# quartiq/stabilizer-stream

Measured on AMD Instinct MI355X. Metric: MS/s ingested (PsdCascade N=1024, raw f32), higher is better.
Workload: dtype f32

## Files before the change

stabilizer-stream_amd/csrc/fused.hip:

```cpp
#include <algorithm>
#include <cmath>
#include <cstdlib>
#include <type_traits>
#include <vector>

#include <hip/hip_ext.h>

#include "fft_block.h"
#include "fft_team.h"
#include "frames.h"
#include "fused_common.h"

#ifndef PSDK_HOIST_LOOKAHEAD
#define PSDK_HOIST_LOOKAHEAD 1
#endif
#ifndef PSDK_UADDR
#define PSDK_UADDR 1
#endif
#ifndef PSDK_ULOOP
#define PSDK_ULOOP 1
#endif

namespace psdk {

#ifdef PSDK_STAMPS
__device__ unsigned long long g_stamps[16];
#define PSDK_STAMP(k)                                                \
    do {                                                             \
        if (stamp_on) {                                              \
            const unsigned long long t_ = __builtin_amdgcn_s_memtime(); \
            st[k] += t_ - tprev;                                     \
            tprev = t_;                                              \
        }                                                            \
    } while (0)
#else
#define PSDK_STAMP(k) \
    do {              \
    } while (0)
#endif

#ifndef PSDK_ABL
#define PSDK_ABL 0
#endif

template <int N>
struct FusedGeo : FusedDec<N> {
    using T = TeamFft<N>;
    static constexpr int TEAM = T::TEAM, TPW = T::TPW;
    static constexpr int TEAMS = FUSED_WAVES * TPW;
    static constexpr int SCR = 2 * T::FRAME;
    static_assert(FusedDec<N>::END <= SCR && FusedDec<N>::WEND <= SCR, "decimator arrays exceed the frame");
    static constexpr size_t LDS_BYTES = sizeof(cf) * (TEAMS * T::FRAME + T::TW0_SIZE + T::TW1_SIZE) +
                                        sizeof(float) * (N + TEAMS * FusedDec<N>::HIST);
};

template <int TEAM>
__device__ __forceinline__ float team_bcast(float v, int team_lane0, int tl)
{
    if constexpr (TEAM == 64)
        return __builtin_bit_cast(float, __builtin_amdgcn_readlane(__builtin_bit_cast(int, v), tl));
    else
        return __shfl(v, team_lane0 + tl, 64);
}

template <class P>
__device__ __forceinline__ P *wave_uniform(P *p)
{
    const uintptr_t a = reinterpret_cast<uintptr_t>(p);
    const unsigned lo = __builtin_amdgcn_readfirstlane((unsigned)a);
    const unsigned hi = __builtin_amdgcn_readfirstlane((unsigned)(a >> 32));
    return reinterpret_cast<P *>((uintptr_t)hi << 32 | lo);
}

__device__ __forceinline__ void addtid_st2(unsigned m0, int dwa, float xa, int dwb, float xb)
{
    unsigned keep;
    asm volatile("s_mov_b32 %0, m0\n\t"
                 "s_mov_b32 m0, %1\n\t"
                 "s_nop 0\n\t"
                 "ds_write_addtid_b32 %2 offset:%4\n\t"
                 "ds_write_addtid_b32 %3 offset:%5\n\t"
                 "s_mov_b32 m0, %0"
                 : "=&s"(keep)
                 : "s"(m0), "v"(xa), "v"(xb), "i"(4 * dwa), "i"(4 * dwb)
                 : "memory");
}

template <int TEAM>
__device__ __forceinline__ float team_sum(float v)
{
    if constexpr (TEAM == 64)
        return wave_sum64(v);
    v = row_sum16(v);
    if constexpr (TEAM == 32)
        v += __shfl_xor(v, 16, 64);
    return v;
}

#ifndef PSDK_EWMA_WPS
#define PSDK_EWMA_WPS FUSED_WAVES_PER_SIMD
#endif
#ifndef PSDK_FOLD
#define PSDK_FOLD 1
#endif
#if PSDK_FOLD
template <int THREADS>
__device__ __forceinline__ void fused_aux_role(const FusedAux &aux, int b, double *scratch)
{
    constexpr int SLICES = 32, BINS = THREADS / SLICES;
    static_assert(BINS == AUX_RED_BINS, "the host sizes the aux grid by AUX_RED_BINS");
    const int n = aux.n, lane = threadIdx.x % BINS, slice = threadIdx.x / BINS;
    const int tall_blocks = aux.nred_tall * aux.red_xb, mid_blocks = aux.nred_mid * aux.red_mb;
    if (b < tall_blocks) {
        const RedJob &job = aux.red[b / aux.red_xb];
        const int k = (b % aux.red_xb) * BINS + lane;
        const bool live = k <= n / 2;
        double acc = 0.0;
        if (live) {
            const int km = k ? n - k : 0;
            int t = slice;
            for (; t + 3 * SLICES < job.nparts; t += 4 * SLICES) {
                float v[4][2];
#pragma unroll
                for (int u = 0; u < 4; ++u) {
                    const float *p = job.partial + (size_t)(t + u * SLICES) * n;
                    v[u][0] = p[k];
                    v[u][1] = p[km];
                }
#pragma unroll
                for (int u = 0; u < 4; ++u)
                    acc += (double)v[u][0] + (double)v[u][1];
            }
            for (; t < job.nparts; t += SLICES) {
                const float *p = job.partial + (size_t)t * n;
                acc += (double)p[k] + (double)p[km];
            }
        }
        scratch[slice * (BINS + 1) + lane] = acc;
        __syncthreads();
        if (slice == 0 && live) {
            acc = 0.0;
#pragma unroll
            for (int i = 0; i < SLICES; ++i)
                acc += scratch[i * (BINS + 1) + lane];
            job.spectrum[k] = job.g_total * job.spectrum[k] + (float)(0.5 * acc);
        }
        return;
    }
    b -= tall_blocks;
    if (b < mid_blocks) {
        const RedJob &job = aux.red[aux.nred_tall + b / aux.red_mb];
        const int g0 = (b % aux.red_mb) * AUX_MID_GROUPS;
        float v[AUX_MID_GROUPS][2][2];
        const bool r0 = slice < job.nparts, r1 = slice + SLICES < job.nparts;
#pragma unroll
        for (int g = 0; g < AUX_MID_GROUPS; ++g) {
            const int k = (g0 + g) * BINS + lane;
            if (k <= n / 2) {
                const int km = k ? n - k : 0;
                if (r0) {
                    v[g][0][0] = job.partial[(size_t)slice * n + k];
                    v[g][0][1] = job.partial[(size_t)slice * n + km];
                }
                if (r1) {
                    v[g][1][0] = job.partial[(size_t)(slice + SLICES) * n + k];
                    v[g][1][1] = job.partial[(size_t)(slice + SLICES) * n + km];
                }
            }
        }
#pragma unroll
        for (int g = 0; g < AUX_MID_GROUPS; ++g) {
            double acc = 0.0;
            if ((g0 + g) * BINS + lane <= n / 2) {
                if (r0)
                    acc += (double)v[g][0][0] + (double)v[g][0][1];
                if (r1)
                    acc += (double)v[g][1][0] + (double)v[g][1][1];
            }
            scratch[(g * SLICES + slice) * (BINS + 1) + lane] = acc;
        }
        __syncthreads();
        const int k = (g0 + slice) * BINS + lane;
        if (slice < AUX_MID_GROUPS && k <= n / 2) {
            double acc = 0.0;
#pragma unroll
            for (int i = 0; i < SLICES; ++i)
                acc += scratch[(slice * SLICES + i) * (BINS + 1) + lane];
            job.spectrum[k] = job.g_total * job.spectrum[k] + (float)(0.5 * acc);
        }
        return;
    }
    b -= mid_blocks;
    if (b < aux.nred - aux.nred_tall - aux.nred_mid) {
        const RedJob &job = aux.red[aux.nred_tall + aux.nred_mid + b];
        for (int k = threadIdx.x; k <= n / 2; k += THREADS) {
            const int km = k ? n - k : 0;
            float v[AUX_SHORT_ROWS][2];
#pragma unroll
            for (int t = 0; t < AUX_SHORT_ROWS; ++t)
                if (t < job.nparts) {
                    v[t][0] = job.partial[(size_t)t * n + k];
                    v[t][1] = job.partial[(size_t)t * n + km];
                }
            double acc = 0.0;
#pragma unroll
            for (int t = 0; t < AUX_SHORT_ROWS; ++t)
                if (t < job.nparts)
                    acc += (double)v[t][0] + (double)v[t][1];
            job.spectrum[k] = job.g_total * job.spectrum[k] + (float)(0.5 * acc);
        }
        return;
    }
    const TailJob &job = aux.tail[b - (aux.nred - aux.nred_tall - aux.nred_mid)];
    for (int i = threadIdx.x; i < job.count; i += THREADS)
        job.dst[i] = job.src[i];
}
#define PSDK_FOLD_PARAM , const FusedAux aux
#ifndef PSDK_AUX_BACK
#define PSDK_AUX_BACK 0
#endif
#ifndef PSDK_PRE_SCOPE
#define PSDK_PRE_SCOPE "workgroup"
#endif
#else
#define PSDK_FOLD_PARAM
#endif

template <int N, int DETREND, bool EWMA, bool FRAMES = false, int SINGLE = 0>
__global__ __launch_bounds__(FUSED_WAVES * 64, EWMA ? PSDK_EWMA_WPS : FUSED_WAVES_PER_SIMD) void fused_kernel(
    const FusedBatch batch, const float *__restrict__ win PSDK_FOLD_PARAM)
{
    using G = FusedGeo<N>;
    using T = TeamFft<N>;
    constexpr int TEAM = G::TEAM, TPW = G::TPW, TEAMS = G::TEAMS;
    __shared__ __attribute__((aligned(16))) cf s_frames[TEAMS * T::FRAME];
    __shared__ cf s_tw0[T::TW0_SIZE];
    __shared__ cf s_tw1[T::TW1_SIZE > 0 ? T::TW1_SIZE : 1];
    __shared__ float4 s_win[N / 4];
    __shared__ float s_hist[TEAMS * G::HIST];

#if PSDK_FOLD
#if PSDK_AUX_BACK
    if ((int)blockIdx.x >= batch.nblocks) {
        fused_aux_role<FUSED_WAVES * 64>(aux, (int)blockIdx.x - batch.nblocks, reinterpret_cast<double *>(s_frames));
        return;
    }
#else
    if ((int)blockIdx.x < aux.nblocks) {
        fused_aux_role<FUSED_WAVES * 64>(aux, (int)blockIdx.x, reinterpret_cast<double *>(s_frames));
        return;
    }
#endif
#endif
#ifdef PSDK_STAMPS
    const unsigned long long t_entry = __builtin_amdgcn_s_memtime();
#endif
    const int tid = threadIdx.x;
    const int lane = tid & 63, wv = tid >> 6;
    const int tm = lane / TEAM, tl = lane % TEAM;
    const int team = wv * TPW + tm;

    for (int i = tid; i < T::TW0_SIZE; i += FUSED_WAVES * 64) {
        const int c = i / TEAM, l = i % TEAM;
        float sn, cs;
        sincospif(-2.0f * (float)(4 * l + c) / (float)N, &sn, &cs);
        s_tw0[i] = {cs, sn};
    }
    for (int i = tid; i < T::TW1_SIZE; i += FUSED_WAVES * 64) {
        const int q = i / 16 + 1, s = i % 16;
        float sn, cs;
        sincospif(-2.0f * (float)(s * q) / (float)T::L1, &sn, &cs);
        s_tw1[i] = {cs, sn};
    }
    for (int i = tid; i < N / 4; i += FUSED_WAVES * 64)
        s_win[i] = *reinterpret_cast<const float4 *>(win + 4 * i);

#if PSDK_FOLD && !PSDK_AUX_BACK
    int bid = (int)blockIdx.x - aux.nblocks;
#else
    int bid = blockIdx.x;
#endif
    if constexpr (FRAMES) {
        for (int g = 0; g < batch.n_fgroups; ++g) {
            const int b0 = batch.fg_begin[g], nb = batch.fg_nb[g];
            if (bid >= b0 && bid < b0 + 4 * nb) {
                const int p = bid - b0, full = (nb >> 3) * 32;
                int c, w;
                if (p < full) {
                    c = (p >> 3) & 3;
                    w = (p >> 5) * 8 + (p & 7);
                } else {
                    const int rem = nb & 7, q_ = p - full;
                    c = q_ / rem;
                    w = (nb & ~7) + q_ % rem;
                }
                bid = b0 + c * nb + w;
                break;
            }
        }
    }
    const int ji = job_of_unit(batch, bid, [](const FusedJob &j) { return j.block_begin; });
    const FusedJob &job = batch.jobs[ji];
    const int wb = bid - job.block_begin;
    const int npairs = job.npairs, run = job.run;
#if PSDK_FOLD
    const bool has_pre = job.pre_count != 0;
    if (has_pre) {
        for (int q = 0; q < job.pre_count; ++q) {
            const TailJob &t = aux.tail[job.pre_first + q];
            for (int i = tid; i < t.count; i += FUSED_WAVES * 64)
                t.dst[i] = t.src[i];
        }
        __builtin_amdgcn_fence(__ATOMIC_RELEASE, PSDK_PRE_SCOPE);
    }
#endif

    cf *frame = s_frames + team * T::FRAME;
    float *sf = reinterpret_cast<float *>(frame);
    float *hs = s_hist + team * G::HIST;
    const unsigned m0f = T::PLANES ? T::lds_base(frame) : 0u;
    if constexpr (T::PLANES) {
        if (T::lds_base(s_frames + (TEAMS - 1) * T::FRAME) >= T::M0_LIMIT)
            __builtin_trap();
    }

    const float ta[HBF_MA] = {PSDK_HBF_TAPS_A};
    const float tb[HBF_MB] = {PSDK_HBF_TAPS_B};
    const float tc[HBF_MC] = {PSDK_HBF_TAPS_C};

    constexpr int HR = (G::HIST + TEAM - 1) / TEAM;
    unsigned h_pack[HR];
#pragma unroll
    for (int r = 0; r < HR; ++r)
        h_pack[r] = G::hist_slot(tl + TEAM * r);

    float q[16];
#pragma unroll
    for (int s = 0; s < 16; ++s)
        q[s] = 0.0f;

    __syncthreads();
#if PSDK_FOLD
    if (has_pre)
        __builtin_amdgcn_fence(__ATOMIC_ACQUIRE, PSDK_PRE_SCOPE);
#endif
#ifdef PSDK_STAMPS
    const bool stamp_on = wb == 0 && run >= 8 && tid < 64;
    unsigned long long st[12] = {0, 0, 0, 0, 0, 0, 0, 0, 0, 0, 0, 0};
    unsigned long long tprev = __builtin_amdgcn_s_memtime();
    st[9] = tprev - t_entry;
#endif

    constexpr bool UNI = TEAM == 64 && !FRAMES;
    constexpr bool UADDR = UNI && PSDK_UADDR != 0, ULOOP = UNI && PSDK_ULOOP != 0;
    const int p0 = ULOOP ? __builtin_amdgcn_readfirstlane((wb * TEAMS + team) * run) : (wb * TEAMS + team) * run;
    const int nrun = min(run, npairs - p0);
    const bool act0 = nrun > 0;
    unsigned voff = UADDR ? 16u * (unsigned)tl : 0u, voff_o = UADDR ? 8u * (unsigned)tl : 0u;
    const float4 *cp = UADDR ? wave_uniform(reinterpret_cast<const float4 *>(job.src) + (size_t)p0 * (N / 4) + N / 4)
                             : reinterpret_cast<const float4 *>(job.src) + (size_t)p0 * (N / 4) + tl;
    auto lane_off = [](unsigned &v) {
        asm volatile("" : "+v"(v));
        return v;
    };
    auto ld4 = [](const float4 *c, int k, unsigned vo) -> float4 {
        typedef float f4v __attribute__((ext_vector_type(4)));
        const f4v r = *(const __attribute__((address_space(1))) f4v *)(reinterpret_cast<const char *>(c + (k - N / 4)) + vo);
        return make_float4(r.x, r.y, r.z, r.w);
    };
    const bool fr = FRAMES && job.fspan >= 0;
    const FrameSpan &fsp = batch.fspans[fr ? job.fspan : 0];
    const unsigned ch_off = fr ? (unsigned)job.fch * 16u : 0u;
    const unsigned dac_flip = (fr && job.fch >= 2) ? 0x80008000u : 0u;
    const __amdgpu_buffer_rsrc_t rsrc = __builtin_amdgcn_make_buffer_rsrc(
        const_cast<uint8_t *>(fsp.frames), 0, fr ? (int)min(fsp.bytes, 0x7FFFFFFFull) : 0, 0x00020000);
    unsigned sp = job.s_off + (unsigned)p0 * N + 4u * tl;
    using G4 = Grp4<FRAMES>;
    auto piece = [&](const float4 *c, unsigned s_, int k) -> G4 {
        G4 g;
        if constexpr (FRAMES) {
            if (fr) {
                const unsigned si = s_ + 4u * (unsigned)k;
                const unsigned off = frame_cell_offset(fsp, si >> 3) + ch_off + (si & 4u) * 2u;
                const auto r = __builtin_amdgcn_raw_buffer_load_b64(rsrc, off, 0, 0);
                g.set_raw((unsigned)r[0], (unsigned)r[1]);
                return g;
            }
        }
        if constexpr (UADDR)
            g.set(ld4(c, k, voff));
        else
            g.set(c[k]);
        return g;
    };
    auto volts = [&](G4 &g) {
        if constexpr (FRAMES) {
            if (fr)
                grp_volts(g, dac_flip, adcdac_lsb());
        }
    };
    const float4 *safe = act0 ? cp : reinterpret_cast<const float4 *>(job.src) + (UADDR ? N / 4 : tl);
    if constexpr (UADDR && !ULOOP)
        safe = wave_uniform(safe);
    unsigned safe_s = act0 ? sp : job.s_off + 4u * tl;
    G4 ga[2], gb[2], gc[2];
    {
        const float4 z4 = make_float4(0.f, 0.f, 0.f, 0.f);
        ga[0].set(z4), ga[1].set(z4), gb[0].set(z4), gb[1].set(z4), gc[0].set(z4), gc[1].set(z4);
    }
    if (act0) {
        ga[0] = piece(cp, sp, 0);
        ga[1] = piece(cp, sp, TEAM);
        gb[0] = piece(cp, sp, 2 * TEAM);
        gb[1] = piece(cp, sp, 3 * TEAM);
        gc[0] = piece(cp, sp, N / 4);
        gc[1] = piece(cp, sp, N / 4 + TEAM);
        volts(ga[0]);
        volts(ga[1]);
        volts(gb[0]);
        volts(gb[1]);
        volts(gc[0]);
        volts(gc[1]);
    }

    {
        const float *xn = job.src + (size_t)p0 * N + N / 2;
        const long long lim = -(long long)job.pre - ((long long)p0 * N + N / 2);
        for (int r = tl; r < G::WX / 2; r += TEAM) {
            const int i0 = 2 * r - G::WX;
            float e = 0.0f, o = 0.0f;
            if (act0 && i0 >= lim) {
                if (fr) {
                    const unsigned long long si = (unsigned long long)((long long)job.s_off + (long long)p0 * N + N / 2 + i0);
                    e = frame_sample(fsp, job.fch, si);
                    o = frame_sample(fsp, job.fch, si + 1);
                } else {
                    e = xn[i0];
                    o = xn[i0 + 1];
                }
            }
            sf[G::WXE + r] = e;
            sf[G::WXO + r] = o;
        }
        wave_sync();
        for (int u = tl; u < G::WA / 2; u += TEAM) {
            float y0, y1;
            hbf_two<HBF_MA, G::A_CE, G::A_CO>(sf + G::WXE, sf + G::WXO, 2 * u, ta, y0, y1);
            sf[G::WAE + u] = y0;
            sf[G::WAO + u] = y1;
            if (u >= G::WA / 2 - 11) {
                hs[u - (G::WA / 2 - 11)] = y0;
                hs[11 + u - (G::WA / 2 - 11)] = y1;
            }
        }
        wave_sync();
        for (int u = tl; u < G::WB / 2; u += TEAM) {
            float y0, y1;
            hbf_two<HBF_MB, G::B_CE, G::B_CO>(sf + G::WAE, sf + G::WAO, 2 * u, tb, y0, y1);
            hs[22 + u] = y0;
            hs[51 + u] = y1;
        }
        wave_sync();
    }

    constexpr bool HREG = HR <= 3;
    float hreg[HR];
#pragma unroll
    for (int r = 0; r < HR; ++r)
        hreg[r] = (HREG && tl + TEAM * r < G::HIST) ? hs[tl + TEAM * r] : 0.0f;
    float piv = 0.0f, s0c = 0.0f;
    if constexpr (DETREND == 3) {
        auto r4 = [](const float4 &x) { return (x.x + x.y) + (x.z + x.w); };
        piv = team_sum<TEAM>((r4(ga[0].f()) + r4(ga[1].f())) + (r4(gb[0].f()) + r4(gb[1].f()))) * (1.0f / (float)N);
        auto s4 = [](const float4 &x, float pv) { return ((x.x - pv) + (x.y - pv)) + ((x.z - pv) + (x.w - pv)); };
        s0c = team_sum<TEAM>(s4(ga[0].f(), piv) + s4(ga[1].f(), piv));
    }
    EwmaAmp eamp;
    if constexpr (EWMA) {
        if (job.ewma)
            eamp.init(job, job.step0 + (SINGLE != 0 ? 1 : 2) * p0);
    }
    PSDK_STAMP(10);
    float keep[16];
#pragma unroll
    for (int s = 0; s < 16; ++s)
        keep[s] = 0.0f;
    auto pair_step = [&](G4(&glo)[2], G4(&gup)[2], G4(&gnl)[2], const float4 *cnext, unsigned snext, bool more,
                         float *o, int p, auto odd_step) {
        constexpr bool DOUBLE = SINGLE == 2, ODD = decltype(odd_step)::value;
        float4 lo[2] = {glo[0].f(), glo[1].f()}, up[2] = {gup[0].f(), gup[1].f()};
        const float4 nl[2] = {gnl[0].f(), gnl[1].f()};
        PSDK_STAMP(0);
#ifdef PSDK_STAMPS
        if constexpr (TEAM == 64) {
            asm volatile("s_waitcnt vmcnt(0)" ::: "memory");
            PSDK_STAMP(1);
        }
#endif
        __builtin_amdgcn_s_setprio(PSDK_DEC_PRIO);
        if constexpr (!(PSDK_ABL & 4)) {
        if constexpr (!(PSDK_ABL & 2)) {
#pragma unroll
        for (int r = 0; r < HR; ++r)
            if ((h_pack[r] & 0xFFFFu) != 0xFFFFu)
                sf[h_pack[r] & 0xFFFFu] = HREG ? hreg[r] : hs[tl + TEAM * r];
        }
        if constexpr (PSDK_ABL & 16) {
        } else if constexpr (TEAM == 64) {
            const float4 *pc[5] = {&lo[1], &up[0], &up[1], &nl[0], &nl[1]};
            float p1y = dpp_shr1(0.0f, pc[0]->y), p1w = dpp_shr1(0.0f, pc[0]->w);
            float p2w = dpp_shr1(0.0f, p1w);
#pragma unroll
            for (int r = 0; r < 4; ++r) {
                const float4 &pv = *pc[r], &cu = *pc[r + 1];
                const float s1x = dpp_shr1(dpp_ror1(pv.x), cu.x), s1y = dpp_shr1(dpp_ror1(pv.y), cu.y);
                const float s1z = dpp_shr1(dpp_ror1(pv.z), cu.z), s1w = dpp_shr1(dpp_ror1(pv.w), cu.w);
                const float s2y = dpp_shr1(dpp_ror1(p1y), s1y), s2w = dpp_shr1(dpp_ror1(p1w), s1w);
                const float s3w = dpp_shr1(dpp_ror1(p2w), s2w);
                float a0 = 0.0f, a1 = 0.0f;
                a0 += (s3w + cu.y) * ta[0];
                a1 += (s2y + cu.w) * ta[0];
                a0 += (s2y + s1w) * ta[1];
                a1 += (s2w + cu.y) * ta[1];
                a0 += (s2w + s1y) * ta[2];
                a1 += (s1y + s1w) * ta[2];
                if constexpr (T::PLANES) {
                    addtid_st2(m0f, G::AE + 11 + TEAM * r, s1x + a0, G::AO + 11 + TEAM * r, s1z + a1);
                } else {
                    const int u = tl + TEAM * r;
                    sf[G::AE + 11 + u] = s1x + a0;
                    sf[G::AO + 11 + u] = s1z + a1;
                }
                p1y = s1y;
                p1w = s1w;
                p2w = s2w;
            }
        } else {
            auto split = [&](int h, const float4 &x) {
                sf[G::XE + h] = x.x;
                sf[G::XE + h + 1] = x.z;
                sf[G::XO + h] = x.y;
                sf[G::XO + h + 1] = x.w;
            };
            if (tl >= TEAM - 3)
                split(2 * (tl - (TEAM - 3)), lo[1]);
            {
                const int h = G::HX / 2 + 2 * tl;
                split(h, up[0]);
                split(h + N / 8, up[1]);
                split(h + N / 4, nl[0]);
                split(h + 3 * N / 8, nl[1]);
            }
            wave_sync();
            PSDK_STAMP(1);
#pragma unroll
            for (int r = 0; r < 2; ++r) {
                const int u = tl + TEAM * r;
                float y[4];
                hbf_four<HBF_MA, G::A_CE, G::A_CO, PSDK_HBF_WIDE_A != 0 && (G::XO % 4 == 0)>(sf + G::XE, sf + G::XO, 4 * u, ta, y);
                sf[G::AE + 11 + 2 * u] = y[0];
                sf[G::AO + 11 + 2 * u] = y[1];
                sf[G::AE + 12 + 2 * u] = y[2];
                sf[G::AO + 12 + 2 * u] = y[3];
            }
        }
        wave_sync();
        PSDK_STAMP(2);
        {
            float y[4];
            hbf_four<HBF_MB, G::B_CE, G::B_CO, PSDK_HBF_WIDE != 0 && (G::AO % 4 == 0)>(sf + G::AE, sf + G::AO, 4 * tl, tb, y);
            sf[G::BE + 29 + 2 * tl] = y[0];
            sf[G::BO + 29 + 2 * tl] = y[1];
            sf[G::BE + 30 + 2 * tl] = y[2];
            sf[G::BO + 30 + 2 * tl] = y[3];
        }
        wave_sync();
        PSDK_STAMP(3);
        if constexpr (!(PSDK_ABL & 32)) {
            float y0, y1;
            hbf_two<HBF_MC, G::C_CE, G::C_CO>(sf + G::BE, sf + G::BO, 2 * tl, tc, y0, y1);
            if ((PSDK_ABL & 1024) ? job.npairs >= 0 : (!(PSDK_ABL & 128) || job.npairs < 0)) {
                if constexpr (PSDK_ABL & 512) {
                    __builtin_nontemporal_store(y0, o + 2 * tl);
                    __builtin_nontemporal_store(y1, o + 2 * tl + 1);
                } else if constexpr (UADDR) {
                    typedef float f2v __attribute__((ext_vector_type(2)));
                    *(__attribute__((address_space(1))) f2v *)(reinterpret_cast<char *>(o) + lane_off(voff_o)) = f2v{y0, y1};
                } else {
                    *reinterpret_cast<f2 *>(o + 2 * tl) = {y0, y1};
                }
            }
        }
        if constexpr (!(PSDK_ABL & 2)) {
#pragma unroll
        for (int r = 0; r < HR; ++r)
            if ((h_pack[r] & 0xFFFFu) != 0xFFFFu)
                (HREG ? hreg[r] : hs[tl + TEAM * r]) = sf[h_pack[r] >> 16];
        }
        }
        wave_sync();
        PSDK_STAMP(4);
        __builtin_amdgcn_s_setprio(0);

        cf v[16];
        {
            DetrendParams dp;
            float &oa = dp.oa, &ob = dp.ob, &ma = dp.ma, &mb = dp.mb;
            slope2 &sa = dp.sa, &sb = dp.sb;
            const int l0 = lane - tl;
            if constexpr (DETREND == 1) {
                oa = team_bcast<TEAM>(up[0].x, l0, 0);
                ob = team_bcast<TEAM>(nl[0].x, l0, 0);
            } else if constexpr (DETREND == 2) {
                oa = team_bcast<TEAM>(lo[0].x, l0, 0);
                sa = span_slope(oa, team_bcast<TEAM>(up[1].w, l0, TEAM - 1), N);
                ob = team_bcast<TEAM>(up[0].x, l0, 0);
                sb = span_slope(ob, team_bcast<TEAM>(nl[1].w, l0, TEAM - 1), N);
            } else if constexpr (DETREND == 3) {
                auto sub4 = [](float4 &x, float pv) {
                    x.x -= pv;
                    x.y -= pv;
                    x.z -= pv;
                    x.w -= pv;
                };
                sub4(lo[0], piv);
                sub4(lo[1], piv);
                sub4(up[0], piv);
                sub4(up[1], piv);
                auto r4 = [](const float4 &x) { return (x.x + x.y) + (x.z + x.w); };
                auto s4 = [](const float4 &x, float pv) { return ((x.x - pv) + (x.y - pv)) + ((x.z - pv) + (x.w - pv)); };
                const float s1 = team_sum<TEAM>(r4(up[0]) + r4(up[1]));
                const float s2 = team_sum<TEAM>(s4(nl[0], piv) + s4(nl[1], piv));
                ob = piv;
                ma = (s0c + s1) * (1.0f / (float)N);
                mb = (s1 + s2) * (1.0f / (float)N);
                const float pnext = piv + mb;
                s0c = fmaf(-(float)(N / 2), pnext - piv, s2);
                piv = pnext;
            }
            if constexpr (EWMA) {
                if (job.ewma) {
                    if constexpr (SINGLE == 0)
                        dp.ea = eamp.next(job);
                    dp.eb = eamp.next(job);
                }
            }
            window_pair<N, DETREND, EWMA, true, SINGLE != 0>(v, tl, lo[0], lo[1], up[0], up[1], nl[0], nl[1], s_win[tl], s_win[TEAM + tl],
                                          s_win[2 * TEAM + tl], s_win[3 * TEAM + tl], dp);
        }
        {
            const float4 *src = more ? cnext : safe;
            if constexpr (UADDR && !ULOOP)
                src = wave_uniform(src);
            const unsigned ssrc = more ? snext : safe_s;
            safe = src;
            safe_s = ssrc;
            if constexpr (!(PSDK_ABL & 64)) {
#if PSDK_HOIST_LOOKAHEAD
            if constexpr (FRAMES) {
                if (fr) {
                    auto fp = [&](G4 &g, int k) {
                        const unsigned si = ssrc + 4u * (unsigned)k;
                        const unsigned off = frame_cell_offset(fsp, si >> 3) + ch_off + (si & 4u) * 2u;
                        const auto r = __builtin_amdgcn_raw_buffer_load_b64(rsrc, off, 0, 0);
                        g.set_raw((unsigned)r[0], (unsigned)r[1]);
                    };
                    fp(gup[0], 2 * TEAM);
                    fp(gup[1], 3 * TEAM);
                    fp(glo[0], N / 4);
                    fp(glo[1], N / 4 + TEAM);
                } else {
                    gup[0].set(src[2 * TEAM]);
                    gup[1].set(src[3 * TEAM]);
                    glo[0].set(src[N / 4]);
                    glo[1].set(src[N / 4 + TEAM]);
                }
            } else if constexpr (UADDR) {
                const unsigned vo = lane_off(voff);
                gup[0].set(ld4(src, 2 * TEAM, vo));
                gup[1].set(ld4(src, 3 * TEAM, vo));
                glo[0].set(ld4(src, N / 4, vo));
                glo[1].set(ld4(src, N / 4 + TEAM, vo));
            } else {
                gup[0].set(src[2 * TEAM]);
                gup[1].set(src[3 * TEAM]);
                glo[0].set(src[N / 4]);
                glo[1].set(src[N / 4 + TEAM]);
            }
#else
            gup[0] = piece(src, ssrc, 2 * TEAM);
            gup[1] = piece(src, ssrc, 3 * TEAM);
            glo[0] = piece(src, ssrc, N / 4);
            glo[1] = piece(src, ssrc, N / 4 + TEAM);
#endif
            }
        }
        PSDK_STAMP(5);
#ifdef PSDK_EXTRA_VALU
        {
            float d[8] = {v[0].re, v[0].im, v[1].re, v[1].im, v[2].re, v[2].im, v[3].re, v[3].im};
#pragma unroll
            for (int e = 0; e < PSDK_EXTRA_VALU; ++e)
                asm volatile("v_fma_f32 %0, %0, %1, %1" : "+v"(d[e & 7]) : "v"(v[4].re));
#pragma unroll
            for (int e = 0; e < 8; ++e)
                asm volatile("" ::"v"(d[e]));
        }
#endif
#ifdef PSDK_EXTRA_LDS
        {
            float d = 0.0f;
#pragma unroll
            for (int e = 0; e < PSDK_EXTRA_LDS; ++e)
                d += lds_ld(frame + 17 * tl + (e & 15)).re;
            asm volatile("" ::"v"(d));
        }
#endif
        if constexpr (DOUBLE && !ODD) {
#pragma unroll
            for (int s = 0; s < 16; ++s)
                keep[s] = v[s].re;
        } else {
        if constexpr (DOUBLE) {
#pragma unroll
            for (int s = 0; s < 16; ++s)
                v[s] = {keep[s], v[s].re};
        }
        T::pass0(tl, v, s_tw0);
        T::template store0<UNI && PSDK_ST0_SINGLE != 0>(tl, v, frame);
        wave_sync();
        PSDK_STAMP(6);
        if constexpr (!(PSDK_ABL & 8)) {
        T::load1(tl, v, frame);
        if constexpr (PSDK_ABL & 1)
            Dft<T::R1>::run(v);
        else
            T::pass1(tl, v, s_tw1);
        if constexpr (T::PLANES)
            T::store1_planes(tl, v, frame, m0f);
        else
            T::store1(tl, v, frame);
        wave_sync();
        PSDK_STAMP(7);
        if constexpr (T::PLANES)
            T::load2_planes(tl, v, frame);
        else
            T::load2(tl, v, frame);
        T::pass2(v);
        }
#pragma unroll
        for (int s = 0; s < 16; ++s)
            q[s] = fmaf(v[s].re, v[s].re, fmaf(v[s].im, v[s].im, q[s]));
        }
        if constexpr (FRAMES) {
            volts(gup[0]);
            volts(gup[1]);
            volts(glo[0]);
            volts(glo[1]);
        }
        wave_sync();
        PSDK_STAMP(8);
    };

    {
        float *o = job.dst + (size_t)p0 * (N / 8);
        if constexpr (UADDR)
            o = wave_uniform(o);
        if constexpr (PSDK_ABL & 2048)
            o = reinterpret_cast<float *>(reinterpret_cast<uintptr_t>(o) & ~(uintptr_t)127);
        for (int i = 0; i < nrun; i += 2) {
            pair_step(ga, gb, gc, cp + N / 4, sp + N, i + 1 < nrun, o, p0 + i, std::false_type{});
            cp += N / 4;
            sp += N;
            if (!(PSDK_ABL & 256))
                o += N / 8;
            if (i + 1 < nrun) {
                pair_step(gc, gb, ga, cp + N / 4, sp + N, i + 2 < nrun, o, p0 + i + 1, std::true_type{});
                cp += N / 4;
                sp += N;
                if (!(PSDK_ABL & 256))
                    o += N / 8;
            }
        }
    }

    PSDK_STAMP(0);
#pragma unroll
    for (int s = 0; s < 16; ++s)
        sf[T::freq_of(tl, s)] = q[s];
    __syncthreads();
    const float *all = reinterpret_cast<const float *>(s_frames);
    float *out = job.partial + (size_t)wb * N;
    for (int k = tid; k < N; k += FUSED_WAVES * 64) {
        float acc = 0.0f;
#pragma unroll
        for (int g = 0; g < TEAMS; ++g)
            acc += all[g * G::SCR + k];
        out[k] = acc;
    }
#ifdef PSDK_STAMPS
    PSDK_STAMP(11);
    if (stamp_on && tid == 0) {
        for (int k = 0; k < 12; ++k)
            g_stamps[k] = st[k];
        g_stamps[12] = (unsigned long long)nrun;
    }
#endif
}

bool fused_supported(int n)
{
    return n == 256 || n == 512 || n == 1024 || n == 2048 || n == 4096 || n == 8192 || n == 16384;
}

bool fused_frames_supported(int n) { return fused_supported(n); }

bool fused_fold_supported(int n) { return PSDK_FOLD != 0 && (n == 256 || n == 512 || n == 1024); }

bool fused_double_supported(int n) { return fused_supported(n); }

int fused_pairs_per_block(int n, int run)
{
    switch (n) {
    case 256:
        return FusedGeo<256>::TEAMS * run;
    case 512:
        return FusedGeo<512>::TEAMS * run;
    case 1024:
        return FusedGeo<1024>::TEAMS * run;
    default:
        return fused_supported(n) ? run : 0;
    }
}

int fused_block_threads(int n) { return n >= 2048 ? n / 16 : FUSED_WAVES * 64; }

int fused_max_blocks(int n)
{
    auto big = [](int threads, int wps) { return 256 * std::max(1, 4 * wps / (threads / 64)); };
    switch (n) {
    case 2048:
        return big(128, BIG_WAVES_PER_SIMD);
    case 4096:
        return big(256, BIG_WAVES_PER_SIMD);
    case 8192:
        return big(512, BIG_WAVES_PER_SIMD);
    case 16384:
        return 256;
    default:
        return 256 * (4 * FUSED_WAVES_PER_SIMD / FUSED_WAVES);
    }
}

template <int N>
static void big_tables_n(std::vector<cf> &tw0, std::vector<cf> &twa)
{
    using T = BlockFft<N>;
    tw0.resize(T::TW0_SIZE);
    twa.resize(T::TWA_SIZE);
    for (int c = 0; c < 4; ++c)
        for (int tl = 0; tl < T::TEAM; ++tl) {
            const double a = -2.0 * M_PI * (double)(4 * tl + c) / (double)N;
            tw0[c * T::TEAM + tl] = {(float)cos(a), (float)sin(a)};
        }
    for (int q = 1; q < T::RA; ++q)
        for (int s2 = 0; s2 < T::SA; ++s2) {
            const double a = -2.0 * M_PI * (double)(s2 * q) / (double)T::L1;
            twa[(q - 1) * T::SA + s2] = {(float)cos(a), (float)sin(a)};
        }
}

void fused_big_tables(int n, std::vector<cf> &tw0, std::vector<cf> &twa)
{
    tw0.clear();
    twa.clear();
    switch (n) {
    case 2048:
        big_tables_n<2048>(tw0, twa);
        break;
    case 4096:
        big_tables_n<4096>(tw0, twa);
        break;
    case 8192:
        big_tables_n<8192>(tw0, twa);
        break;
    case 16384:
        big_tables_n<16384>(tw0, twa);
        break;
    default:
        break;
    }
}

void fused_big3_table(int n, std::vector<cf> &tw3)
{
    tw3.clear();
    if (n != 2048 && n != 4096)
        return;
    const int team = n / 16;
    tw3.resize(2 * (size_t)team);
    for (int tl = 0; tl < team; ++tl) {
        const double a = -2.0 * M_PI * (double)tl / (double)n;
        tw3[tl] = {(float)cos(a), (float)sin(a)};
        tw3[team + tl] = {(float)cos(4.0 * a), (float)sin(4.0 * a)};
    }
}

template <int N>
static hipError_t launch_fused_n(const FusedBatch &b, const float *win, hipStream_t s, hipEvent_t ea, hipEvent_t eb, const FusedAux *auxp)
{
#if PSDK_FOLD
    static const FusedAux no_aux{};
    const FusedAux &aux = auxp ? *auxp : no_aux;
#define PSDK_FOLD_ARG , aux
#else
    (void)auxp;
#define PSDK_FOLD_ARG
#endif

    static_assert(FusedGeo<N>::LDS_BYTES * (4 * FUSED_WAVES_PER_SIMD / FUSED_WAVES) <= 163840,
                  "the workgroups of a CU (two of eight waves by default) share its 160 KiB of LDS");
#if PSDK_FOLD
    const dim3 grid(b.nblocks + aux.nblocks), block(FUSED_WAVES * 64);
#else
    const dim3 grid(b.nblocks), block(FUSED_WAVES * 64);
#endif
    const bool ew_ = b.any_ewma, frm_ = b.any_frames;
#define PSDK_FUSED_CASE(D)                                                                \
    case D:                                                                               \
        if (frm_ && ew_)                                                                  \
            hipExtLaunchKernelGGL((fused_kernel<N, D, true, true>), grid, block, 0, s, ea, eb, 0, b, win PSDK_FOLD_ARG);  \
        else if (frm_)                                                                    \
            hipExtLaunchKernelGGL((fused_kernel<N, D, false, true>), grid, block, 0, s, ea, eb, 0, b, win PSDK_FOLD_ARG); \
        else if (ew_)                                                                     \
            hipExtLaunchKernelGGL((fused_kernel<N, D, true>), grid, block, 0, s, ea, eb, 0, b, win PSDK_FOLD_ARG);  \
        else                                                                              \
            hipExtLaunchKernelGGL((fused_kernel<N, D, false>), grid, block, 0, s, ea, eb, 0, b, win PSDK_FOLD_ARG); \
        break;
#define PSDK_FUSED_SINGLE(D)                                                                              \
    case D:                                                                                               \
        if (b.single == 2 && ew_)                                                                         \
            hipExtLaunchKernelGGL((fused_kernel<N, D, true, false, 2>), grid, block, 0, s, ea, eb, 0, b, win PSDK_FOLD_ARG);  \
        else if (b.single == 2)                                                                           \
            hipExtLaunchKernelGGL((fused_kernel<N, D, false, false, 2>), grid, block, 0, s, ea, eb, 0, b, win PSDK_FOLD_ARG); \
        else if (ew_)                                                                                     \
            hipExtLaunchKernelGGL((fused_kernel<N, D, true, false, 1>), grid, block, 0, s, ea, eb, 0, b, win PSDK_FOLD_ARG);  \
        else                                                                                              \
            hipExtLaunchKernelGGL((fused_kernel<N, D, false, false, 1>), grid, block, 0, s, ea, eb, 0, b, win PSDK_FOLD_ARG); \
        break;
    if (b.single) {
        if (b.any_frames)
            return hipErrorInvalidValue;
        switch (b.detrend) {
            PSDK_FUSED_SINGLE(0)
            PSDK_FUSED_SINGLE(1)
            PSDK_FUSED_SINGLE(2)
            PSDK_FUSED_SINGLE(3)
        default:
            return hipErrorInvalidValue;
        }
        return hipGetLastError();
    }
#undef PSDK_FUSED_SINGLE
    switch (b.detrend) {
        PSDK_FUSED_CASE(0)
        PSDK_FUSED_CASE(1)
        PSDK_FUSED_CASE(2)
        PSDK_FUSED_CASE(3)
    default:
        return hipErrorInvalidValue;
    }
#undef PSDK_FUSED_CASE
    return hipGetLastError();
}

hipError_t launch_bigfused_2048(const FusedBatch &, const float *, const cf *, const cf *, hipStream_t, hipEvent_t, hipEvent_t);
hipError_t launch_bigfused_4096(const FusedBatch &, const float *, const cf *, const cf *, hipStream_t, hipEvent_t, hipEvent_t);
hipError_t launch_bigfused_8192(const FusedBatch &, const float *, const cf *, const cf *, hipStream_t, hipEvent_t, hipEvent_t);
hipError_t launch_bigfused_16384(const FusedBatch &, const float *, const cf *, const cf *, hipStream_t, hipEvent_t, hipEvent_t);
hipError_t launch_bigfused3_2048(const FusedBatch &, const float *, const cf *, hipStream_t, hipEvent_t, hipEvent_t);
hipError_t launch_bigfused3_4096(const FusedBatch &, const float *, const cf *, hipStream_t, hipEvent_t, hipEvent_t);

hipError_t launch_fused(int n, const FusedBatch &b, const float *win, const cf *tw0g, const cf *twag, const cf *tw3g, hipStream_t s,
                        hipEvent_t ea, hipEvent_t eb, const FusedAux *aux)
{
    if (b.nblocks <= 0)
        return hipSuccess;
    if (tw3g) {
        if (n == 2048)
            return launch_bigfused3_2048(b, win, tw3g, s, ea, eb);
        if (n == 4096)
            return launch_bigfused3_4096(b, win, tw3g, s, ea, eb);
    }
    switch (n) {
    case 256:
        return launch_fused_n<256>(b, win, s, ea, eb, aux);
    case 512:
        return launch_fused_n<512>(b, win, s, ea, eb, aux);
    case 1024:
        return launch_fused_n<1024>(b, win, s, ea, eb, aux);
    case 2048:
        return launch_bigfused_2048(b, win, tw0g, twag, s, ea, eb);
    case 4096:
        return launch_bigfused_4096(b, win, tw0g, twag, s, ea, eb);
    case 8192:
        return launch_bigfused_8192(b, win, tw0g, twag, s, ea, eb);
    case 16384:
        return launch_bigfused_16384(b, win, tw0g, twag, s, ea, eb);
    default:
        return hipErrorInvalidValue;
    }
}

}

#ifdef PSDK_STAMPS
extern "C" int psdc_debug_stamps(unsigned long long *out16)
{
    return (int)hipMemcpyFromSymbol(out16, HIP_SYMBOL(psdk::g_stamps), 16 * sizeof(unsigned long long));
}
#endif
```

stabilizer-stream_amd/csrc/fused_common.h:

```cpp
#pragma once
#include <hip/hip_runtime.h>

#include "fft_core.h"
#include "hbf_taps.h"
#include "kernels.h"

#ifndef PSDK_HBF_WIDE
#define PSDK_HBF_WIDE 1
#endif
#ifndef PSDK_XO_PAD
#define PSDK_XO_PAD 0
#endif
#ifndef PSDK_HBF_WIDE_A
#define PSDK_HBF_WIDE_A 0
#endif
#ifndef PSDK_DEC_PRIO
#define PSDK_DEC_PRIO 3
#endif

namespace psdk {

template <int N, bool NOX = false>
struct FusedDec {
    static constexpr int HX = 12, HA = 22, HB = 58;
    static constexpr int XE = 0, XO = XE + HX / 2 + N / 2 + (N >= 2048 ? PSDK_XO_PAD : 0);
    static constexpr int AE = NOX ? 0 : XO + HX / 2 + N / 2, AO = AE + 12 + N / 4;
    static constexpr int BE = AO + 12 + N / 4, BO = BE + 30 + N / 8;
    static constexpr int END = BO + 30 + N / 8;
    static constexpr int HIST = HA + HB;
    static constexpr int WX = HBF_HALO, WA = HBF_PRE_A, WB = HBF_PRE_B;
    static constexpr int WXE = 0, WXO = WX / 2, WAE = WX, WAO = WX + WA / 2 + 1;
    static constexpr int WEND = WAO + WA / 2 + 1;
    static constexpr int A_CE = 4, A_CO = 1, B_CE = 6, B_CO = 0, C_CE = 15, C_CO = 0;
    static_assert(HX / 2 - 2 == A_CE && HX / 2 - 5 == A_CO, "x history vs stage A offsets");
    static_assert(HA / 2 - 5 == B_CE && HA / 2 - 11 == B_CO, "A history vs stage B offsets");
    static_assert(HB / 2 - 14 == C_CE && HB / 2 - 29 == C_CO, "B history vs stage C offsets");
    static_assert(WX / 2 - WA - HBF_MA + 1 == A_CE && WA / 2 - WB - HBF_MB + 1 == B_CE, "warm-up geometry");

    static __device__ __forceinline__ unsigned hist_slot(int i)
    {
        int front = -1, shift = 0;
        if (i < 11) {
            front = AE + i;
            shift = N / 4;
        } else if (i < 22) {
            front = AO + (i - 11);
            shift = N / 4;
        } else if (i < 51) {
            front = BE + (i - 22);
            shift = N / 8;
        } else if (i < 80) {
            front = BO + (i - 51);
            shift = N / 8;
        }
        return front < 0 ? 0xFFFFu : ((unsigned)(front + shift) << 16) | (unsigned)front;
    }
};

__device__ __forceinline__ void wave_sync()
{
    __builtin_amdgcn_fence(__ATOMIC_RELEASE, "wavefront");
    __builtin_amdgcn_wave_barrier();
    __builtin_amdgcn_fence(__ATOMIC_ACQUIRE, "wavefront");
}

__device__ __forceinline__ float dpp_shr1(float fill, float v)
{
    return __builtin_bit_cast(float, __builtin_amdgcn_update_dpp(__builtin_bit_cast(int, fill),
                                                                 __builtin_bit_cast(int, v), 0x138, 0xf, 0xf, false));
}
__device__ __forceinline__ float dpp_ror1(float v)
{
    return __builtin_bit_cast(float, __builtin_amdgcn_mov_dpp(__builtin_bit_cast(int, v), 0x13C, 0xf, 0xf, false));
}

__device__ __forceinline__ float row_sum16(float v)
{
#define PSDK_DPP(x, ctrl) \
    __builtin_bit_cast(float, __builtin_amdgcn_update_dpp(0, __builtin_bit_cast(int, (x)), (ctrl), 0xf, 0xf, true))
    v += PSDK_DPP(v, 0xB1);
    v += PSDK_DPP(v, 0x4E);
    v += PSDK_DPP(v, 0x141);
    v += PSDK_DPP(v, 0x140);
#undef PSDK_DPP
    return v;
}
template <int W>
__device__ __forceinline__ float group_sum(float v)
{
    static_assert(W == 1 || W == 2 || W == 4 || W == 8 || W == 16, "group of lanes within a row");
#define PSDK_DPP(x, ctrl) \
    __builtin_bit_cast(float, __builtin_amdgcn_update_dpp(0, __builtin_bit_cast(int, (x)), (ctrl), 0xf, 0xf, true))
    if constexpr (W >= 2)
        v += PSDK_DPP(v, 0xB1);
    if constexpr (W >= 4)
        v += PSDK_DPP(v, 0x4E);
    if constexpr (W >= 8)
        v += PSDK_DPP(v, 0x141);
    if constexpr (W >= 16)
        v += PSDK_DPP(v, 0x140);
#undef PSDK_DPP
    return v;
}
__device__ __forceinline__ float wave_sum64(float v)
{
    const int b = __builtin_bit_cast(int, row_sum16(v));
    const float r0 = __builtin_bit_cast(float, __builtin_amdgcn_readlane(b, 0));
    const float r1 = __builtin_bit_cast(float, __builtin_amdgcn_readlane(b, 16));
    const float r2 = __builtin_bit_cast(float, __builtin_amdgcn_readlane(b, 32));
    const float r3 = __builtin_bit_cast(float, __builtin_amdgcn_readlane(b, 48));
    return (r0 + r1) + (r2 + r3);
}

struct f2 {
    float x, y;
};

template <bool FRAMES>
struct Grp4;
template <>
struct Grp4<false> {
    float4 v;
    __device__ __forceinline__ float4 f() const { return v; }
    __device__ __forceinline__ void set(const float4 &x) { v = x; }
};
template <>
struct Grp4<true> {
    unsigned x, y, z, w;
    __device__ __forceinline__ float4 f() const
    {
        return make_float4(__builtin_bit_cast(float, x), __builtin_bit_cast(float, y), __builtin_bit_cast(float, z),
                           __builtin_bit_cast(float, w));
    }
    __device__ __forceinline__ void set(const float4 &v)
    {
        x = __builtin_bit_cast(unsigned, v.x), y = __builtin_bit_cast(unsigned, v.y);
        z = __builtin_bit_cast(unsigned, v.z), w = __builtin_bit_cast(unsigned, v.w);
    }
    __device__ __forceinline__ void set_raw(unsigned a, unsigned b) { x = a, y = b, z = 0u, w = 0u; }
};
__device__ __forceinline__ void grp_volts(Grp4<true> &g, unsigned flip, float lsb)
{
    const unsigned a = g.x ^ flip, b = g.y ^ flip;
    g.set(make_float4((float)(short)(unsigned short)(a & 0xffffu) * lsb, (float)(short)(unsigned short)(a >> 16) * lsb,
                      (float)(short)(unsigned short)(b & 0xffffu) * lsb, (float)(short)(unsigned short)(b >> 16) * lsb));
}
__device__ __forceinline__ f2 ld2(const float *p)
{
    const cf v = lds_ld(reinterpret_cast<const cf *>(p));
    return {v.re, v.im};
}

template <int M, int CE, int CO>
__device__ __forceinline__ void hbf_two(const float *__restrict__ ev, const float *__restrict__ od, int j,
                                        const float (&taps)[M], float &y0, float &y1)
{
    constexpr int LO = CO & ~1;
    constexpr int CNT = (CO - LO) + 2 * M + 1;
    constexpr int NP = (CNT + 1) / 2;
    float w[2 * NP];
#pragma unroll
    for (int k = 0; k < NP; ++k) {
        const f2 v = ld2(od + j + LO + 2 * k);
        w[2 * k] = v.x;
        w[2 * k + 1] = v.y;
    }
    constexpr int O = CO - LO;
    float a0 = 0.0f, a1 = 0.0f;
#pragma unroll
    for (int i = 0; i < M; ++i) {
        a0 += (w[O + i] + w[O + 2 * M - 1 - i]) * taps[i];
        a1 += (w[O + 1 + i] + w[O + 2 * M - i]) * taps[i];
    }
    float e0, e1;
    if constexpr ((CE & 1) == 0) {
        const f2 e = ld2(ev + j + CE);
        e0 = e.x;
        e1 = e.y;
    } else {
        e0 = ev[j + CE];
        e1 = ev[j + CE + 1];
    }
    y0 = e0 + a0;
    y1 = e1 + a1;
}

template <int M, int CE, int CO, bool WIDE = false>
__device__ __forceinline__ void hbf_four(const float *__restrict__ ev, const float *__restrict__ od, int j,
                                         const float (&taps)[M], float (&y)[4])
{
    constexpr int LO = WIDE ? (CO & ~3) : (CO & ~1);
    constexpr int CNT = (CO - LO) + 2 * M + 3;
    constexpr int NP = WIDE ? 2 * ((CNT + 3) / 4) : (CNT + 1) / 2;
    float w[2 * NP];
    if constexpr (WIDE) {
#pragma unroll
        for (int k = 0; k < NP / 2; ++k) {
            typedef float f4v __attribute__((ext_vector_type(4)));
            const f4v v = *(const volatile __attribute__((address_space(3))) f4v *)(od + j + LO + 4 * k);
            w[4 * k] = v.x, w[4 * k + 1] = v.y, w[4 * k + 2] = v.z, w[4 * k + 3] = v.w;
        }
    } else {
#pragma unroll
        for (int k = 0; k < NP; ++k) {
            const f2 v = ld2(od + j + LO + 2 * k);
            w[2 * k] = v.x;
            w[2 * k + 1] = v.y;
        }
    }
    constexpr int O = CO - LO;
    float a[4] = {0.0f, 0.0f, 0.0f, 0.0f};
#pragma unroll
    for (int i = 0; i < M; ++i)
#pragma unroll
        for (int t = 0; t < 4; ++t)
            a[t] += (w[O + t + i] + w[O + t + 2 * M - 1 - i]) * taps[i];
    float e[4];
    if constexpr ((CE & 1) == 0) {
        const f2 e01 = ld2(ev + j + CE), e23 = ld2(ev + j + CE + 2);
        e[0] = e01.x, e[1] = e01.y, e[2] = e23.x, e[3] = e23.y;
    } else {
        const f2 e12 = ld2(ev + j + CE + 1);
        e[0] = ev[j + CE], e[1] = e12.x, e[2] = e12.y, e[3] = ev[j + CE + 3];
    }
#pragma unroll
    for (int t = 0; t < 4; ++t)
        y[t] = e[t] + a[t];
}

__device__ __forceinline__ float fused_ewma_amp(const FusedJob &job, int step)
{
    const int m = step > job.is_m1 ? step : job.is_m1;
    const int na = job.nb - m;
    if (na <= 0)
        return 1.0f;
    return (float)exp2(0.5 * (double)na * job.log2_gamma);
}

struct EwmaAmp {
    double a = 1.0, rho = 1.0;
    int step = 0;
    bool zero = false;
    __device__ __forceinline__ void init(const FusedJob &job, int s)
    {
        step = s;
        zero = !(job.log2_gamma > -1.0e300);
        rho = zero ? 0.0 : exp2(-0.5 * job.log2_gamma);
        const int m = s > job.is_m1 ? s : job.is_m1;
        const int na = job.nb - m;
        a = na <= 0 ? 1.0 : (zero ? 0.0 : exp2(0.5 * (double)na * job.log2_gamma));
    }
    __device__ __forceinline__ float next(const FusedJob &job)
    {
        const float r = (float)a;
        if (step >= job.is_m1 && step < job.nb) {
            if (step + 1 >= job.nb)
                a = 1.0;
            else if (!zero)
                a *= rho;
        }
        ++step;
        return r;
    }
};

struct DetrendParams {
    float oa = 0.0f, ob = 0.0f, ma = 0.0f, mb = 0.0f;
    slope2 sa = {0.0f, 0.0f}, sb = {0.0f, 0.0f};
    float ea = 1.0f, eb = 1.0f;
};
template <int N, int DETREND, bool EWMA, bool CENTRED = false, bool SINGLE = false>
__device__ __forceinline__ void window_pair(cf (&v)[16], int tl, const float4 &lo0, const float4 &lo1, const float4 &up0,
                                            const float4 &up1, const float4 &nl0, const float4 &nl1, const float4 &w0,
                                            const float4 &w1, const float4 &w2, const float4 &w3, const DetrendParams &d)
{
    const float nf = (float)(4 * tl);
    auto put = [&](int slot, float xa, float xb, float w, int nofs) {
        if constexpr (DETREND == 1) {
            xa -= d.oa;
            xb -= d.ob;
        } else if constexpr (DETREND == 2) {
            const float n = nf + (float)nofs;
            xa = fmaf(-n, d.sa.lo, fmaf(-n, d.sa.hi, xa - d.oa));
            xb = fmaf(-n, d.sb.lo, fmaf(-n, d.sb.hi, xb - d.ob));
        } else if constexpr (DETREND == 3 && CENTRED) {
            xa -= d.ma;
            xb = slot < 8 ? xb - d.mb : (xb - d.ob) - d.mb;
        } else if constexpr (DETREND == 3) {
            xa = (xa - d.oa) - d.ma;
            xb = (xb - d.ob) - d.mb;
        }
        xa *= w;
        xb *= w;
        if constexpr (EWMA) {
            xa *= d.ea;
            xb *= d.eb;
        }
        if constexpr (SINGLE)
            v[slot] = {xb, 0.0f};
        else
            v[slot] = {xa, xb};
    };
    put(0, lo0.x, up0.x, w0.x, 0);
    put(1, lo0.y, up0.y, w0.y, 1);
    put(2, lo0.z, up0.z, w0.z, 2);
    put(3, lo0.w, up0.w, w0.w, 3);
    put(4, lo1.x, up1.x, w1.x, N / 4);
    put(5, lo1.y, up1.y, w1.y, N / 4 + 1);
    put(6, lo1.z, up1.z, w1.z, N / 4 + 2);
    put(7, lo1.w, up1.w, w1.w, N / 4 + 3);
    put(8, up0.x, nl0.x, w2.x, N / 2);
    put(9, up0.y, nl0.y, w2.y, N / 2 + 1);
    put(10, up0.z, nl0.z, w2.z, N / 2 + 2);
    put(11, up0.w, nl0.w, w2.w, N / 2 + 3);
    put(12, up1.x, nl1.x, w3.x, 3 * N / 4);
    put(13, up1.y, nl1.y, w3.y, 3 * N / 4 + 1);
    put(14, up1.z, nl1.z, w3.z, 3 * N / 4 + 2);
    put(15, up1.w, nl1.w, w3.w, 3 * N / 4 + 3);
}

}
```

Baseline: 737,400.

## Peel odd pair, single-exit pair loop, late lookahead loads, nofill DPP shifts

Restructures the per-wave pair loop so an odd leading pair is peeled and the main loop runs full pairs with one exit test. The lookahead global loads are moved into a lambda and issued after pass0 behind a scheduling barrier, which shortens their register live range and sets where they overlap with compute. DPP shift-right for the carry values drops the explicit zero fill, saving a move per shift. The aim is to cut loop-control branching and register pressure. The risk is a different latency-hiding profile, and lanes without a fill may carry stale values if the zero was ever relied on.

```diff
diff --git a/stabilizer-stream_amd/csrc/fused.hip b/stabilizer-stream_amd/csrc/fused.hip
--- a/stabilizer-stream_amd/csrc/fused.hip
+++ b/stabilizer-stream_amd/csrc/fused.hip
@@ -19,6 +19,12 @@
 #endif
 #ifndef PSDK_ULOOP
 #define PSDK_ULOOP 1
+#endif
+#ifndef PSDK_LOOP_1EXIT
+#define PSDK_LOOP_1EXIT 1
+#endif
+#ifndef PSDK_DPP_NOZERO
+#define PSDK_DPP_NOZERO 1
 #endif
 
 namespace psdk {
@@ -353,6 +359,7 @@
 
     constexpr bool UNI = TEAM == 64 && !FRAMES;
     constexpr bool UADDR = UNI && PSDK_UADDR != 0, ULOOP = UNI && PSDK_ULOOP != 0;
+    constexpr bool LOOP2 = PSDK_LOOP_1EXIT != 0 && UNI && !EWMA && DETREND <= 1;
     const int p0 = ULOOP ? __builtin_amdgcn_readfirstlane((wb * TEAMS + team) * run) : (wb * TEAMS + team) * run;
     const int nrun = min(run, npairs - p0);
     const bool act0 = nrun > 0;
@@ -508,8 +515,13 @@
         if constexpr (PSDK_ABL & 16) {
         } else if constexpr (TEAM == 64) {
             const float4 *pc[5] = {&lo[1], &up[0], &up[1], &nl[0], &nl[1]};
+#if PSDK_DPP_NOZERO
+            float p1y = dpp_shr1_nofill(pc[0]->y), p1w = dpp_shr1_nofill(pc[0]->w);
+            float p2w = dpp_shr1_nofill(p1w);
+#else
             float p1y = dpp_shr1(0.0f, pc[0]->y), p1w = dpp_shr1(0.0f, pc[0]->w);
             float p2w = dpp_shr1(0.0f, p1w);
+#endif
 #pragma unroll
             for (int r = 0; r < 4; ++r) {
                 const float4 &pv = *pc[r], &cu = *pc[r + 1];
@@ -648,6 +660,9 @@
             window_pair<N, DETREND, EWMA, true, SINGLE != 0>(v, tl, lo[0], lo[1], up[0], up[1], nl[0], nl[1], s_win[tl], s_win[TEAM + tl],
                                           s_win[2 * TEAM + tl], s_win[3 * TEAM + tl], dp);
         }
+#if PSDK_LOOP_1EXIT
+        auto lookahead = [&]
+#endif
         {
             const float4 *src = more ? cnext : safe;
             if constexpr (UADDR && !ULOOP)
@@ -695,6 +710,12 @@
 #endif
             }
         }
+#if PSDK_LOOP_1EXIT
+        ;
+        constexpr bool LA_LATE = LOOP2 && !(SINGLE == 2 && !decltype(odd_step)::value);
+        if constexpr (!LA_LATE)
+            lookahead();
+#endif
         PSDK_STAMP(5);
 #ifdef PSDK_EXTRA_VALU
         {
@@ -727,6 +748,12 @@
                 v[s] = {keep[s], v[s].re};
         }
         T::pass0(tl, v, s_tw0);
+#if PSDK_LOOP_1EXIT
+        if constexpr (LA_LATE) {
+            __builtin_amdgcn_sched_barrier(0x84);
+            lookahead();
+        }
+#endif
         T::template store0<UNI && PSDK_ST0_SINGLE != 0>(tl, v, frame);
         wave_sync();
         PSDK_STAMP(6);
@@ -768,6 +795,32 @@
             o = wave_uniform(o);
         if constexpr (PSDK_ABL & 2048)
             o = reinterpret_cast<float *>(reinterpret_cast<uintptr_t>(o) & ~(uintptr_t)127);
+        if constexpr (LOOP2) {
+        auto advance = [&] {
+            cp += N / 4;
+            sp += N;
+            if (!(PSDK_ABL & 256))
+                o += N / 8;
+        };
+        int i = 0;
+        if (act0 && (nrun & 1)) {
+            pair_step(ga, gb, gc, cp + N / 4, sp + N, nrun > 1, o, p0, std::false_type{});
+            advance();
+#pragma unroll
+            for (int h = 0; h < 2; ++h) {
+                const G4 t = ga[h];
+                ga[h] = gc[h];
+                gc[h] = t;
+            }
+            i = 1;
+        }
+        for (; i + 1 < nrun; i += 2) {
+            pair_step(ga, gb, gc, cp + N / 4, sp + N, true, o, p0 + i, std::false_type{});
+            advance();
+            pair_step(gc, gb, ga, cp + N / 4, sp + N, i + 2 < nrun, o, p0 + i + 1, std::true_type{});
+            advance();
+        }
+        } else
         for (int i = 0; i < nrun; i += 2) {
             pair_step(ga, gb, gc, cp + N / 4, sp + N, i + 1 < nrun, o, p0 + i, std::false_type{});
             cp += N / 4;
diff --git a/stabilizer-stream_amd/csrc/fused_common.h b/stabilizer-stream_amd/csrc/fused_common.h
--- a/stabilizer-stream_amd/csrc/fused_common.h
+++ b/stabilizer-stream_amd/csrc/fused_common.h
@@ -72,6 +72,11 @@
 __device__ __forceinline__ float dpp_ror1(float v)
 {
     return __builtin_bit_cast(float, __builtin_amdgcn_mov_dpp(__builtin_bit_cast(int, v), 0x13C, 0xf, 0xf, false));
+}
+
+__device__ __forceinline__ float dpp_shr1_nofill(float v)
+{
+    return __builtin_bit_cast(float, __builtin_amdgcn_mov_dpp(__builtin_bit_cast(int, v), 0x138, 0xf, 0xf, false));
 }
 
 __device__ __forceinline__ float row_sum16(float v)
```

Result: no change. 741,500, median of 6 (+0.6%).
